# pscoro/JPEG-XL-Lossy-Image-Compression-Thesis

Hardware: AMD Instinct MI355X
Metric: MPix/s VarDCT encode @ d1.0, 8K RGB (higher is better)
Workload: dtype f32; 1 GPU; 8k 7680x4320 RGB8 (synth_rgb8), VarDCT d1 e7, cjxl defaults (JXG_FLAGS_CJXL_DEFAULTS: Gaborish + EPF + masking AQ), proposals=0, ans-coded, 1 frame(s) per step, 2 distinct frames cycled, streaming entry points (jxg_submit_rgb8_device / jxg_receive, one host thread); global_batch=1, parallelism=frame-dp1

## Files before the change

jpeg-xl-lossy-image-compression-thesis_amd/csrc/jxg_ac.hip:

```cpp
#include "jxg_device.h"
#include "jxg_kernels.h"

namespace jxg {

constexpr int kAcCtxPad = (kAcCtx + 15) & ~15;
__constant__ __attribute__((aligned(16))) uint8_t c_cluster[kAcCtxPad];

constexpr int kAcThreads = 1024;

struct GroupGeom {
  int bx0, by0, gw, gh;
};
__device__ __forceinline__ uint32_t slot_group(const uint32_t* glist, uint32_t g0, uint32_t i) {
  return glist ? glist[i] : g0 + i;
}
__device__ __forceinline__ GroupGeom group_geom(const AcArgs& a, int g) {
  GroupGeom r;
  const int gx = g % (int)a.gxs, gy = g / (int)a.gxs;
  r.bx0 = gx * 32;
  r.by0 = gy * 32;
  r.gw = min(32, (int)a.bxs - r.bx0);
  r.gh = min(32, (int)a.bys - r.by0);
  return r;
}

__device__ __forceinline__ void load_coefs(const int16_t* q, uint32_t* w) {
  const uint4* p = reinterpret_cast<const uint4*>(q);
#pragma unroll
  for (int i = 0; i < 8; i++) {
    const uint4 t = p[i];
    w[4 * i + 0] = t.x;
    w[4 * i + 1] = t.y;
    w[4 * i + 2] = t.z;
    w[4 * i + 3] = t.w;
  }
}
__device__ __forceinline__ int32_t coef(const uint32_t* w, int k) {
  return (int32_t)(int16_t)(w[k >> 1] >> ((k & 1) * 16));
}

__device__ __forceinline__ int freq_ctx(int k) {
  return k < 16 ? max(k - 1, 0) : (k < 32 ? 15 + ((k - 16) >> 1) : 23 + ((k - 32) >> 2));
}
__device__ __forceinline__ int nnz_ctx(int n) {
  return n < 2 ? 0 : n < 3 ? 31 : n < 5 ? 62 : n < 9 ? 93 : n < 13 ? 123 : n < 21 ? 152
       : n < 33 ? 180 : 206;
}

__device__ __forceinline__ int block_ctx_of(int c, int acs) {
  return kDefaultCtxMap[(c < 2 ? c ^ 1 : 2) * 13 + kStrategyOrder[acs]];
}

constexpr int kAcTok = 64;
constexpr int kEmitLdsWords = 24576;

__device__ __forceinline__ int channel_of(int ci) { return ci == 0 ? 1 : (ci == 1 ? 0 : 2); }

__device__ __forceinline__ void varblock_dims(int type, int& lcb, int& cx, int& cy) {
  switch (type) {
    case 6: lcb = 1, cx = 1, cy = 2; break;
    case 7: lcb = 1, cx = 2, cy = 1; break;
    case 4: lcb = 2, cx = 2, cy = 2; break;
    case 10: lcb = 3, cx = 2, cy = 4; break;
    case 11: lcb = 3, cx = 4, cy = 2; break;
    case 5: lcb = 4, cx = 4, cy = 4; break;
    case 19: lcb = 5, cx = 4, cy = 8; break;
    case 20: lcb = 5, cx = 8, cy = 4; break;
    case 18: lcb = 6, cx = 8, cy = 8; break;
    case 22: lcb = 7, cx = 8, cy = 16; break;
    case 23: lcb = 7, cx = 16, cy = 8; break;
    case 21: lcb = 8, cx = 16, cy = 16; break;
    case 25: lcb = 9, cx = 16, cy = 32; break;
    case 26: lcb = 9, cx = 32, cy = 16; break;
    case 24: lcb = 10, cx = 32, cy = 32; break;
    default: lcb = 0, cx = 1, cy = 1; break;
  }
}

constexpr int kBands = 4;
static_assert(kBands * kBandTokStride == kGroupTokStride, "band record spaces tile the group's");

__device__ __forceinline__ uint32_t rec_index(const uint32_t* bt, uint32_t k) {
  uint32_t j = 0, lo = 0, cum = 0;
#pragma unroll
  for (int i = 0; i < kBands - 1; i++) {
    cum += bt[i];
    const bool past = k >= cum;
    lo = past ? cum : lo;
    j += past ? 1u : 0u;
  }
  return j * (uint32_t)kBandTokStride + (k - lo);
}

struct SliceTask {
  bool valid;
  int bx, by, obx, oby, sl, lcb, cx, type;
  size_t gb, ogb;
};
__device__ __forceinline__ SliceTask slice_task(const AcArgs& a, const GroupGeom& G, int y0) {
  SliceTask t;
  const int b = threadIdx.x;
  t.bx = b & 31;
  t.by = y0 + (b >> 5);
  t.valid = t.bx < G.gw && t.by < G.gh;
  if (!t.valid) t.bx = t.by = 0;
  t.gb = (size_t)(G.by0 + t.by) * a.bxs + G.bx0 + t.bx;
  t.type = t.valid ? (a.acs[t.gb] & 0x7F) : 0;
  int cy;
  varblock_dims(t.type, t.lcb, t.cx, cy);
  t.obx = t.bx & ~(t.cx - 1);
  t.oby = t.by & ~(cy - 1);
  t.sl = (t.by - t.oby) * t.cx + (t.bx - t.obx);
  t.ogb = (size_t)(G.by0 + t.oby) * a.bxs + G.bx0 + t.obx;
  return t;
}
__device__ __forceinline__ int block_of_slice(const SliceTask& t, int j, int y0) {
  return (t.oby - y0 + j / t.cx) * 32 + t.obx + j % t.cx;
}

template <int BR>
struct AcLds {
  uint8_t nz[3][(BR + 1) * 32];
  uint8_t snz[3][BR * 32];
  uint8_t last[3][BR * 32];
  int8_t lastk[3][BR * 32];
};
__device__ __forceinline__ int predict_nz(const uint8_t* nzc, int bx, int by, int y0) {
  const int r = by - y0 + 1;
  if (bx == 0) return by == 0 ? 32 : nzc[(r - 1) * 32 + bx];
  if (by == 0) return nzc[r * 32 + bx - 1];
  return (nzc[(r - 1) * 32 + bx] + nzc[r * 32 + bx - 1] + 1) / 2;
}

template <int BR>
__device__ __forceinline__ uint32_t task_token_count(const AcArgs& a, const SliceTask& t,
                                                     const AcLds<BR>& L, int c, int y0) {
  if (t.lcb == 0) {
    uint32_t w[32];
    load_coefs(a.ac + (t.gb * 3 + c) * 64, w);
    int last = 0;
#pragma unroll
    for (int kk = 1; kk < 64; kk++) last = coef(w, kk) != 0 ? kk : last;
    return 1u + (uint32_t)last;
  }
  const int cb = 1 << t.lcb;
  int K = -1;
  for (int j = 0; j < cb; j++) {
    const int lk = L.lastk[c][block_of_slice(t, j, y0)];
    K = lk >= 0 ? j * 64 + lk : K;
  }
  const int lo = max(t.sl * 64, cb), hi = min(t.sl * 64 + 63, K);
  return (t.sl == 0 ? 1u : 0u) + (hi >= lo ? (uint32_t)(hi - lo + 1) : 0u);
}

template <int BR>
__device__ __forceinline__ void fill_slices(const AcArgs& a, const GroupGeom& G,
                                            const SliceTask& t, AcLds<BR>& L, int y0) {
  const size_t nb = (size_t)a.bxs * a.bys;
  constexpr int kPos = (BR + 1) * 32, kNT = BR * 32, kIt = (kPos + kNT - 1) / kNT;
  uint32_t acsv[kIt], nzv[kIt][3];
  bool in[kIt];
#pragma unroll
  for (int it = 0; it < kIt; it++) {
    const int i = threadIdx.x + it * kNT, r = i >> 5, bx = i & 31, by = y0 - 1 + r;
    in[it] = i < kPos && bx < G.gw && by >= 0 && by < G.gh;
    const size_t gb = in[it] ? (size_t)(G.by0 + by) * a.bxs + G.bx0 + bx : 0;
    acsv[it] = in[it] ? a.acs[gb] : 0u;
#pragma unroll
    for (int c = 0; c < 3; c++) nzv[it][c] = in[it] ? a.nz[c * nb + gb] : 0u;
  }
#pragma unroll
  for (int it = 0; it < kIt; it++) {
    if (!in[it]) continue;
    const int i = threadIdx.x + it * kNT;
    int l, cx, cy;
    varblock_dims((int)acsv[it], l, cx, cy);
#pragma unroll
    for (int c = 0; c < 3; c++) L.nz[c][i] = (uint8_t)((nzv[it][c] + (1u << l) - 1) >> l);
  }
  if (t.valid && t.lcb > 0) {
    const int cb = 1 << t.lcb, me = threadIdx.x;
#pragma unroll 1
    for (int c = 0; c < 3; c++) {
      uint32_t w[32];
      load_coefs(a.ac + (t.gb * 3 + c) * 64, w);
      int n = 0, lk = -1;
#pragma unroll
      for (int kk = 0; kk < 64; kk++) {
        const bool on = (t.sl * 64 + kk >= cb) && coef(w, kk) != 0;
        n += on;
        lk = on ? kk : lk;
      }
      L.snz[c][me] = (uint8_t)n;
      L.last[c][me] = coef(w, 63) != 0;
      L.lastk[c][me] = (int8_t)lk;
    }
  }
}

template <int BR>
__device__ __forceinline__ void slice_state(const SliceTask& t, const AcLds<BR>& L, int c, int y0,
                                            int nz, int& left, int& prev) {
  const int cb = 1 << t.lcb;
  left = nz;
  prev = nz > cb * 4 ? 0 : 1;
  if (t.sl > 0) {
    for (int j = 0; j < t.sl; j++) left -= L.snz[c][block_of_slice(t, j, y0)];
    if (t.sl * 64 - 1 >= cb) prev = L.last[c][block_of_slice(t, t.sl - 1, y0)];
  }
}

template <int NT>
__device__ __forceinline__ uint32_t block_excl_scan(uint32_t v, uint32_t* sWave,
                                                    uint32_t* total) {
  const int lane = threadIdx.x & 63, wv = threadIdx.x >> 6;
  uint32_t incl = v;
#pragma unroll
  for (int d = 1; d < 64; d <<= 1) {
    const uint32_t t = __shfl_up(incl, d);
    if (lane >= d) incl += t;
  }
  if (lane == 63) sWave[wv] = incl;
  __syncthreads();
  uint32_t before = 0, all = 0;
#pragma unroll
  for (int i = 0; i < NT / 64; i++) {
    const uint32_t x = sWave[i];
    before += i < wv ? x : 0u;
    all += x;
  }
  *total = all;
  return before + incl - v;
}

#ifdef JXG_FRONT_PROFILE
__device__ unsigned long long g_hprof[8];
#define HPROF(k)                                                     \
  do {                                                               \
    if (threadIdx.x == 0) {                                          \
      const unsigned long long now_ = __builtin_readcyclecounter();  \
      if ((k) > 0) atomicAdd(&g_hprof[(k)], now_ - hprof_t0);       \
      else atomicAdd(&g_hprof[0], 1ull);                             \
      hprof_t0 = now_;                                               \
    }                                                                \
  } while (0)
void dump_hist_profile() {
  unsigned long long h[8];
  if (hipMemcpyFromSymbol(h, HIP_SYMBOL(g_hprof), sizeof(h)) != hipSuccess) return;
  static const char* kNames[6] = {"workgroups", "fill slices", "token counts", "scan", "walk", "flush"};
  std::fprintf(stderr, "ac_hist thread-0 shader cycles (Mcycles summed over workgroups):\n");
  for (int k = 0; k < 6; k++) std::fprintf(stderr, "  %-16s %12.3f\n", kNames[k], k ? h[k] / 1e6 : (double)h[0]);
}
#else
#define HPROF(k) \
  do {           \
  } while (0)
void dump_hist_profile() {}
#endif
template <int BR>
__global__ __launch_bounds__(BR * 32) void ac_hist_kernel(Batch<AcArgs> bt_) {
  constexpr int kBandBlocks = BR * 32, kHistThreads = kBandBlocks, kWgBands = 32 / BR;
  const AcArgs& a = bt_.a[blockIdx.z];
  constexpr bool kWide = BR == 32;
  constexpr int kHistWords = kWide ? kMaxClusters * kAcTok : kMaxClusters * kAcTok / 2;
  __shared__ uint32_t sHist[kHistWords];
  __shared__ AcLds<BR> L;
  __shared__ __attribute__((aligned(16))) uint8_t sClu[kAcCtxPad];
  __shared__ uint32_t sTask[3][kBandBlocks];
  __shared__ uint32_t sBase[kBandBlocks];
  __shared__ uint32_t sWave[kHistThreads / 64];
  __shared__ uint32_t sBound, sNtok[3];
  __shared__ uint16_t sNnzCtx[64];
  __shared__ uint8_t sFreqCtx[64];
  const uint32_t slot = blockIdx.x / kWgBands, band = blockIdx.x % kWgBands;
  const int g = (int)slot_group(a.glist, a.g0, slot);
  const GroupGeom G = group_geom(a, g);
  const int y0 = (int)band * BR;
  if (BR == 32 && threadIdx.x > 0 && threadIdx.x < kBands)
    a.bandtok[g * kBands + threadIdx.x] = 0;
  if (y0 >= G.gh) {
    if (threadIdx.x == 0) a.bandtok[g * kBands + band] = 0;
    return;
  }
#ifdef JXG_FRONT_PROFILE
  unsigned long long hprof_t0 = 0;
#endif
  HPROF(0);
  for (int i = threadIdx.x; i < kHistWords; i += blockDim.x) sHist[i] = 0;
  if (threadIdx.x < 64) {
    sNnzCtx[threadIdx.x] = (uint16_t)nnz_ctx(threadIdx.x);
    sFreqCtx[threadIdx.x] = (uint8_t)freq_ctx(threadIdx.x);
  }
  {
    constexpr int kQ = kAcCtxPad / 16, kQIt = (kQ + kHistThreads - 1) / kHistThreads;
    uint4 q[kQIt];
#pragma unroll
    for (int it = 0; it < kQIt; it++) {
      const int i = threadIdx.x + it * kHistThreads;
      q[it] = i < kQ ? reinterpret_cast<const uint4*>(c_cluster)[i] : make_uint4(0, 0, 0, 0);
    }
#pragma unroll
    for (int it = 0; it < kQIt; it++) {
      const int i = threadIdx.x + it * kHistThreads;
      if (i < kQ) reinterpret_cast<uint4*>(sClu)[i] = q[it];
    }
  }
  if (threadIdx.x < 3) sNtok[threadIdx.x] = 0;
  if (threadIdx.x == 0) sBound = 0;
  const SliceTask t = slice_task(a, G, y0);
  uint32_t nzo[3];
#pragma unroll
  for (int c = 0; c < 3; c++) nzo[c] = t.valid ? a.nz[c * (size_t)a.bxs * a.bys + t.ogb] : 0u;
  fill_slices(a, G, t, L, y0);
  __syncthreads();
  HPROF(1);
  const int me = threadIdx.x;
  if (t.valid) {
#pragma unroll 1
    for (int ci = 0; ci < 3; ci++) sTask[ci][me] = task_token_count(a, t, L, channel_of(ci), y0);
  }
  __syncthreads();
  HPROF(2);
  uint32_t vtot = 0;
  const int cb = 1 << t.lcb;
  if (t.valid && t.sl == 0) {
    for (int ci = 0; ci < 3; ci++)
      for (int j = 0; j < cb; j++) vtot += sTask[ci][block_of_slice(t, j, y0)];
  }
  uint32_t total;
  const uint32_t off = block_excl_scan<kHistThreads>(vtot, sWave, &total);
  if (t.valid && t.sl == 0) sBase[me] = off;
  __syncthreads();
  HPROF(3);
  uint32_t bound = 0, nt[3] = {0, 0, 0};
  uint32_t* rec = a.tokens + (uint64_t)slot * kGroupTokStride + (uint64_t)band * kBandTokStride;
  uint32_t pos = t.valid ? sBase[(t.oby - y0) * 32 + t.obx] : 0u;
  const int lane = threadIdx.x & 63;
  const uint64_t below = lane ? (~0ull >> (64 - lane)) : 0ull;
  auto hist_add = [&](uint32_t clu, uint32_t tok) {
    const uint32_t bin = clu * kAcTok + tok;
    if (kWide)
      atomicAdd(&sHist[bin], 1u);
    else
      atomicAdd(&sHist[bin >> 1], 1u << ((bin & 1u) * 16u));
  };
#pragma unroll 1
  for (int ci = 0; ci < 3; ci++) {
    const int c = channel_of(ci);
    uint32_t idx = 0, cnt = 0, info = 0, info2 = 0, tok0 = 0;
    if (t.valid) {
      uint32_t before = 0, chan_total = 0;
      for (int j = 0; j < cb; j++) {
        const uint32_t b = sTask[ci][block_of_slice(t, j, y0)];
        before += j < t.sl ? b : 0u;
        chan_total += b;
      }
      idx = pos + before;
      cnt = sTask[ci][me];
      pos += chan_total;
      const int nz = (int)nzo[c];
      int left, prev;
      slice_state(t, L, c, y0, nz, left, prev);
      const int bctx = block_ctx_of(c, t.type);
      info = (uint32_t)left | ((uint32_t)prev << 16) | ((uint32_t)t.lcb << 17) |
             ((uint32_t)bctx << 21);
      info2 = (uint32_t)t.sl;
      if (t.sl == 0) {
        const int pred = predict_nz(L.nz[c], t.bx, t.by, y0);
        uint32_t tok, nb, bits;
        hybrid420((uint32_t)nz, tok, nb, bits);
        const uint32_t clu = sClu[nz_bucket(pred) * kBlockCtx + bctx];
        hist_add(clu, tok);
        bound += 15u + nb;
        tok0 = clu | (tok << 8) | (nb << 14) | (bits << 18);
        rec[idx] = tok0;
      }
      nt[0] += c == 0 ? cnt : 0u;
      nt[1] += c == 1 ? cnt : 0u;
      nt[2] += c == 2 ? cnt : 0u;
    }
    const bool need = t.valid && cnt > (t.sl == 0 ? 1u : 0u);
    const uint32_t qoff = (uint32_t)((t.gb * 3 + c) * 64);
    uint64_t M = __ballot(need);
#ifndef JXG_AC_BATCH
#define JXG_AC_BATCH 8
#endif
    constexpr int kBatch = JXG_AC_BATCH;
    while (M) {
      int js[kBatch];
#pragma unroll
      for (int u = 0; u < kBatch; u++) {
        js[u] = M ? (int)__builtin_ctzll(M) : -1;
        M = M ? M & (M - 1) : 0ull;
      }
      int32_t v8[kBatch];
#pragma unroll
      for (int u = 0; u < kBatch; u++)
        v8[u] = js[u] >= 0 ? a.ac[(uint32_t)__builtin_amdgcn_readlane((int)qoff, js[u]) + lane] : 0;
#pragma unroll
      for (int u = 0; u < kBatch; u++) {
        if (js[u] < 0) break;
        const int j = js[u];
        const uint32_t ij = (uint32_t)__builtin_amdgcn_readlane((int)info, j);
        const uint32_t idxj = (uint32_t)__builtin_amdgcn_readlane((int)idx, j);
        const int slj = __builtin_amdgcn_readlane((int)info2, j), lcbj = (ij >> 17) & 15;
        const int leftj = ij & 0xFFFF, prevj = (ij >> 16) & 1, bctxj = ij >> 21;
        const int cbj = 1 << lcbj;
        const int k = slj * 64 + lane;
        const int lo = max(slj * 64, cbj);
        const int32_t v = v8[u];
        const bool on = k >= cbj;
        const uint64_t m = __ballot(on && v != 0);
        const int left_k = leftj - __popcll(m & below);
        if (on && left_k > 0) {
          const int prev_k = k == lo ? prevj : (int)((m >> (lane - 1)) & 1);
          const int ctx = kBlockCtx * kNzBuckets + kZdCtx * bctxj +
                          (sNnzCtx[(left_k + cbj - 1) >> lcbj] + sFreqCtx[k >> lcbj]) * 2 + prev_k;
          uint32_t tok, nb, bits;
          hybrid420(pack_signed(v), tok, nb, bits);
          const uint32_t clu = sClu[ctx];
          hist_add(clu, tok);
          bound += 15u + nb;
          rec[idxj + (slj == 0 ? 1u : 0u) + (uint32_t)(k - lo)] =
              clu | (tok << 8) | (nb << 14) | (bits << 18);
        }
      }
    }
  }
  atomicAdd(&sBound, bound);
  atomicAdd(&sNtok[0], nt[0]);
  atomicAdd(&sNtok[1], nt[1]);
  atomicAdd(&sNtok[2], nt[2]);
  __syncthreads();
  HPROF(4);
  for (int i = threadIdx.x; i < kHistWords; i += blockDim.x) {
    const uint32_t w = sHist[i];
    if (!w) continue;
    if (kWide) {
      atomicAdd(&a.hist[(i / kAcTok) * kAlpha + (i % kAcTok)], w);
      continue;
    }
    const int bin = 2 * i;
    if (w & 0xFFFFu) atomicAdd(&a.hist[(bin / kAcTok) * kAlpha + (bin % kAcTok)], w & 0xFFFFu);
    if (w >> 16) atomicAdd(&a.hist[((bin + 1) / kAcTok) * kAlpha + ((bin + 1) % kAcTok)], w >> 16);
  }
  if (threadIdx.x == 0) {
    atomicAdd(&a.bound[g], sBound);
    atomicAdd(&a.ntok[g * 3 + 0], sNtok[0]);
    atomicAdd(&a.ntok[g * 3 + 1], sNtok[1]);
    atomicAdd(&a.ntok[g * 3 + 2], sNtok[2]);
    a.bandtok[g * kBands + band] = total;
  }
  HPROF(5);
}

__device__ __forceinline__ uint32_t wave_incl_scan(uint32_t v) {
  const int lane = threadIdx.x & 63;
#pragma unroll
  for (int d = 1; d < 64; d <<= 1) {
    const uint32_t t = __shfl_up(v, d);
    if (lane >= d) v += t;
  }
  return v;
}
__global__ __launch_bounds__(kAcThreads) void ac_emit_kernel(AcArgs a) {
  __shared__ uint32_t sCode[kMaxClusters * kAcTok];
  __shared__ __attribute__((aligned(16))) uint32_t sBits[kEmitLdsWords];
  __shared__ uint32_t sWave[kAcThreads / 64];
  const int g = (int)slot_group(a.glist, a.g0, blockIdx.x);
  for (int i = threadIdx.x; i < kMaxClusters * kAcTok; i += blockDim.x)
    sCode[i] = a.codes[(i / kAcTok) * kAlpha + (i % kAcTok)];
  for (int i = threadIdx.x; i < kEmitLdsWords / 4; i += blockDim.x)
    reinterpret_cast<uint4*>(sBits)[i] = make_uint4(0, 0, 0, 0);
  const uint32_t n = a.ntok[g * 3] + a.ntok[g * 3 + 1] + a.ntok[g * 3 + 2];
  const uint32_t* rec = a.tokens + (uint64_t)blockIdx.x * kGroupTokStride;
  uint32_t bt[kBands];
#pragma unroll
  for (int i = 0; i < kBands; i++) bt[i] = a.bandtok[g * kBands + i];
  constexpr int kWaves = kAcThreads / 64;
  const int lane = threadIdx.x & 63, wv = threadIdx.x >> 6;
  const uint32_t chunk = ((n + kWaves * 64 - 1) / (kWaves * 64)) * 64;
  const uint32_t lo = min(n, wv * chunk), hi = min(n, lo + chunk);
  __syncthreads();
  auto code_of = [&](uint32_t r) { return sCode[(r & 0xFF) * kAcTok + ((r >> 8) & 63)]; };
  uint32_t tot = 0;
  for (uint32_t k = lo + lane; k < hi; k += 64) {
    const uint32_t r = rec[rec_index(bt, k)];
    tot += (code_of(r) >> 16) + ((r >> 14) & 15);
  }
#pragma unroll
  for (int d = 32; d > 0; d >>= 1) tot += __shfl_xor(tot, d, 64);
  if (lane == 0) sWave[wv] = tot;
  __syncthreads();
  uint32_t run = 0, total = 0;
#pragma unroll
  for (int i = 0; i < kWaves; i++) {
    const uint32_t x = sWave[i];
    run += i < wv ? x : 0u;
    total += x;
  }
  const uint64_t base = a.base[g];
  const bool lds = total <= (uint32_t)kEmitLdsWords * 32u;
  if (!lds) {
    for (uint32_t i = threadIdx.x; i < (total + 31) / 32; i += blockDim.x) a.scratch[(base >> 5) + i] = 0;
    __threadfence();
    __syncthreads();
  }
  uint32_t* buf = lds ? sBits : a.scratch;
  const uint64_t bias = lds ? 0 : base;
  for (uint32_t k0 = lo; k0 < hi; k0 += 64) {
    const uint32_t k = k0 + lane;
    uint32_t len = 0, val = 0;
    if (k < hi) {
      const uint32_t r = rec[rec_index(bt, k)], cl = code_of(r);
      len = (cl >> 16) + ((r >> 14) & 15);
      val = (cl & 0xFFFFu) | ((r >> 18) << (cl >> 16));
    }
    const uint32_t incl = wave_incl_scan(len);
    if (len) {
      const uint64_t pos = bias + run + incl - len;
      const uint64_t w = pos >> 5;
      const uint32_t sh = (uint32_t)(pos & 31);
      atomicOr(&buf[w], val << sh);
      if (sh + len > 32) atomicOr(&buf[w + 1], val >> (32 - sh));
    }
    run += __shfl(incl, 63, 64);
  }
  if (lds) {
    __syncthreads();
    const uint32_t nw = (total + 31) / 32;
    uint32_t* dst = a.scratch + (base >> 5);
    for (uint32_t i = threadIdx.x; i < nw; i += blockDim.x) dst[i] = sBits[i];
  }
  if (threadIdx.x == 0) a.bits[g] = total;
}

constexpr int kAnsWgWaves = 8;
constexpr int kAnsHelpers = 6;
constexpr int kAnsPieces = (64 + kAnsHelpers - 1) / kAnsHelpers;
constexpr int kAnsBlk = 64;
constexpr int kAnsRow = 65;
constexpr uint32_t kAnsIdle = kAnsHists * 64;
struct AnsConst {
  double rcp;
  uint32_t nf2;
  uint32_t base2;
};
struct AnsChainP {
  int n;
  uint32_t slot;
  uint32_t c1, c2, c3;
  uint32_t g;
  uint32_t pad[2];
};
struct AnsLds {
  AnsConst c[kAnsIdle + 1];
  uint16_t ent[256];
  uint32_t inv[kAnsHists * 4096 / 2];
  uint32_t ea[2][kAnsBlk * kAnsRow];
  uint32_t x[2][kAnsBlk * kAnsRow];
  AnsChainP ch[64];
  int T;
};
__device__ __forceinline__ void ans_chain(const AnsArgs& a, uint32_t blk) {
  __shared__ __attribute__((aligned(16))) AnsLds L;
  const uint32_t c0 = blk * 64;
  if (c0 >= a.n) return;
  const uint32_t* src = reinterpret_cast<const uint32_t*>(a.tab);
  for (uint32_t i = threadIdx.x; i < a.nhist * 512; i += blockDim.x)
    reinterpret_cast<uint4*>(L.inv)[i] = reinterpret_cast<const uint4*>(src + kAnsInvOff / 4)[i];
  for (uint32_t i = threadIdx.x; i <= kAnsIdle; i += blockDim.x) {
    uint32_t f = 4096, row = 0;
    if (i < a.nhist * 64) {
      const uint32_t e = src[(i >> 6) * 128 + (i & 63)];
      f = (e & 0xFFF) + 1;
      row = (i >> 6) * 4096 + (e >> 12);
    }
    L.c[i].rcp = 1.0 / (double)f;
    L.c[i].nf2 = (uint32_t)(-(int)(2 * f));
    L.c[i].base2 = 2 * row;
  }
  for (uint32_t i = threadIdx.x; i < 256; i += blockDim.x)
    L.ent[i] = (uint16_t)(i < 136 ? min((uint32_t)a.tab[kAnsMapOff + i], kAnsHists - 1) * 64 * 16
                                  : kAnsIdle * 16);
  const uint32_t lane = threadIdx.x & 63, wave = threadIdx.x >> 6;
  if (wave == 0) {
    AnsChainP P = {0, 0, 0, 0, 0, ~0u, {0, 0}};
    if (c0 + lane < a.n) {
      P.slot = a.order[c0 + lane];
      P.g = slot_group(a.glist, a.g0, P.slot);
      P.n = (int)(a.ntok[P.g * 3] + a.ntok[P.g * 3 + 1] + a.ntok[P.g * 3 + 2]);
      P.c1 = a.bandtok[P.g * kBands];
      P.c2 = P.c1 + a.bandtok[P.g * kBands + 1];
      P.c3 = P.c2 + a.bandtok[P.g * kBands + 2];
    }
    L.ch[lane] = P;
    int m = P.n;
#pragma unroll
    for (int d = 32; d > 0; d >>= 1) m = max(m, __shfl_xor(m, d, 64));
    if (lane == 0) L.T = m + 1;
  }
  __syncthreads();
  const int NB = (L.T + kAnsBlk - 1) / kAnsBlk;
  const uint8_t* inv = reinterpret_cast<const uint8_t*>(L.inv);
  const uint8_t* cst = reinterpret_cast<const uint8_t*>(L.c);
  const int h = (wave & 3) ? (int)(wave >> 2) * 3 + (int)(wave & 3) - 1 : -1;
  const uint32_t hs = lane;
  auto word_of = [&](uint32_t rec) {
    return ((uint32_t)L.ent[rec & 0xFF] + ((rec >> 4) & 0x3F0)) | ((rec >> 14) & 15) | (rec >> 18) << 14;
  };
  auto record = [&](const AnsChainP& P, int i) {
    const uint32_t u = (uint32_t)i;
    const uint32_t j = (u >= P.c1 ? 1u : 0u) + (u >= P.c2 ? 1u : 0u) + (u >= P.c3 ? 1u : 0u);
    const uint32_t lo = u >= P.c3 ? P.c3 : u >= P.c2 ? P.c2 : u >= P.c1 ? P.c1 : 0u;
    return a.tokens[(uint64_t)P.slot * kGroupTokStride + j * (uint32_t)kBandTokStride + (u - lo)];
  };
  constexpr uint32_t kIdleRec = 0xFFu;
  auto fetch = [&](int b, uint32_t* R) {
#pragma unroll
    for (int j = 0; j < kAnsPieces; j++) {
      const int q = h + kAnsHelpers * j;
      R[j] = kIdleRec;
      if (q < 64) {
        const AnsChainP P = L.ch[q];
        const int i = P.n - 1 - (b * kAnsBlk + (int)hs);
        if (i >= 0) R[j] = record(P, i);
      }
    }
  };
  auto fill = [&](int b, const uint32_t* R) {
#pragma unroll
    for (int j = 0; j < kAnsPieces; j++) {
      const int q = h + kAnsHelpers * j;
      if (q < 64) L.ea[b & 1][hs * kAnsRow + q] = word_of(R[j]);
    }
  };
  auto unstage = [&](int b, uint32_t* X, uint32_t* RC) {
#pragma unroll
    for (int j = 0; j < kAnsPieces; j++) {
      const int q = h + kAnsHelpers * j;
      X[j] = RC[j] = 0;
      if (q < 64) {
        X[j] = L.x[b & 1][hs * kAnsRow + q];
        RC[j] = L.ea[b & 1][hs * kAnsRow + q];
      }
    }
  };
  auto flush = [&](int b, const uint32_t* X, const uint32_t* RC) {
#pragma unroll
    for (int j = 0; j < kAnsPieces; j++) {
      const int q = h + kAnsHelpers * j;
      if (q < 64) {
        const AnsChainP P = L.ch[q];
        const int i = P.n - 1 - (b * kAnsBlk + (int)hs);
        const uint32_t x = X[j], w = RC[j];
        if (i >= 0) {
          const uint32_t nf2 = reinterpret_cast<const AnsConst*>(cst + (w & 0x3FF0))->nf2;
          const bool em = (x >> 12) >= (uint32_t)__mul24((int)nf2, -128);
          const uint32_t raw = w >> 14, nb = w & 15;
          const uint64_t o = (uint64_t)P.slot * kGroupTokStride + (uint32_t)i;
          a.val[o] = em ? (x & 0xFFFFu) | raw << 16 : raw;
          a.len[o] = (uint8_t)(em ? nb + 16 : nb);
        } else if (i == -1 && P.g != ~0u) {
          a.state[P.g] = x;
        }
      }
    }
  };
  uint32_t k = 0x130u, v = 0;
  auto chain_block = [&](int b) {
    const uint32_t* eas = L.ea[b & 1] + lane;
    uint32_t* xo = L.x[b & 1] + lane;
    AnsConst Cn = *reinterpret_cast<const AnsConst*>(cst + (eas[0] & 0x3FF0));
#pragma unroll
    for (int s = 0; s < kAnsBlk; s++) {
      const AnsConst C = Cn;
      if (s + 1 < kAnsBlk) Cn = *reinterpret_cast<const AnsConst*>(cst + (eas[(s + 1) * kAnsRow] & 0x3FF0));
      const double hr = 0.5 * C.rcp;
      const uint32_t Fq = (uint32_t)__mul24((int)C.nf2, -128);
      const uint32_t sh = k >= Fq ? 16u : 0u;
      const uint32_t x = (k << 12) + v;
      const uint32_t xs = x >> sh;
      const uint32_t kk = (uint32_t)__builtin_fma((double)xs, C.rcp, hr);
      const uint32_t x2 = (xs << 1) + C.base2;
      uint32_t addr;
      asm("v_mad_i32_i24 %0, %1, %2, %3" : "=v"(addr) : "v"(kk), "v"(C.nf2), "v"(x2));
      v = *reinterpret_cast<const uint16_t*>(inv + addr);
      k = kk;
      xo[s * kAnsRow] = x;
    }
  };
  if (wave == 0) __builtin_amdgcn_s_setprio(3);
  uint32_t R[kAnsPieces], X[kAnsPieces], RC[kAnsPieces];
  if (h >= 0) {
    fetch(0, R);
    fill(0, R);
    fetch(1, R);
  }
  __syncthreads();
  for (int b = 0; b < NB; b++) {
    if (wave == 0) {
      chain_block(b);
    } else if (h >= 0) {
      if (b > 0) unstage(b - 1, X, RC);
      fill(b + 1, R);
      fetch(b + 2, R);
      if (b > 0) flush(b - 1, X, RC);
    }
    __syncthreads();
  }
  if (h >= 0) {
    unstage(NB - 1, X, RC);
    flush(NB - 1, X, RC);
  }
}
__global__ __launch_bounds__(kAnsWgWaves * 64) void ans_encode_kernel(Batch<AnsArgs> bt_) {
  ans_chain(bt_.a[blockIdx.z], blockIdx.x);
}
constexpr int kAnsDiagWaves = 8;
__device__ __forceinline__ uint32_t wave_ror1(uint32_t x) {
  return (uint32_t)__builtin_amdgcn_mov_dpp((int)x, 0x13C, 0xF, 0xF, false);
}
__device__ __forceinline__ void ans_chain_diag(const AnsArgs& a, uint32_t blk) {
  __shared__ uint32_t sSym[kAnsHists * 128];
  __shared__ uint32_t sInv[kAnsHists * 4096 / 2];
  __shared__ uint8_t sMap[136];
  const uint32_t* src = reinterpret_cast<const uint32_t*>(a.tab);
  for (uint32_t i = threadIdx.x; i < a.nhist * 128; i += blockDim.x) sSym[i] = src[i];
  for (uint32_t i = threadIdx.x; i < a.nhist * 2048; i += blockDim.x)
    sInv[i] = src[kAnsInvOff / 4 + i];
  for (uint32_t i = threadIdx.x; i < 136; i += blockDim.x) sMap[i] = a.tab[kAnsMapOff + i];
  __syncthreads();
  const uint8_t* inv = reinterpret_cast<const uint8_t*>(sInv);
  const uint32_t lane = threadIdx.x & 63;
  const uint32_t gi = __builtin_amdgcn_readfirstlane(blk * kAnsDiagWaves + (threadIdx.x >> 6));
  if (gi >= a.n) return;
  const uint32_t slot = __builtin_amdgcn_readfirstlane(a.order[gi]);
  const uint32_t g = __builtin_amdgcn_readfirstlane(slot_group(a.glist, a.g0, slot));
  __builtin_amdgcn_s_setprio(3);
  const int n = (int)(a.ntok[g * 3] + a.ntok[g * 3 + 1] + a.ntok[g * 3 + 2]);
  const uint64_t b = (uint64_t)slot * kGroupTokStride;
  uint32_t bt[kBands];
#pragma unroll
  for (int i = 0; i < kBands; i++) bt[i] = a.bandtok[g * kBands + i];
  uint32_t k = 0x130u, v = 0;
  uint32_t rec = (int)lane < min(64, n) ? a.tokens[b + rec_index(bt, n - 1 - lane)] : 0u;
  for (int hi = n; hi > 0; hi -= 64) {
    const int cnt = min(64, hi);
    uint32_t f = 4096, base2 = 0;
    if ((int)lane < cnt) {
      const uint32_t h = sMap[rec & 0xFF], e = sSym[h * 128 + ((rec >> 8) & 63)];
      f = (e & 0xFFF) + 1;
      base2 = 2 * (h * 4096 + (e >> 12));
    }
    const uint32_t Fq = f << 8;
    const uint32_t nf2 = (uint32_t)(-(int)(2 * f));
    const double rcp = 1.0 / (double)f, hr = 0.5 * rcp;
    const int hn = hi - 64;
    const uint32_t nrec = (int)lane < min(64, hn) ? a.tokens[b + rec_index(bt, hn - 1 - lane)] : 0u;
    uint32_t X = 0;
    uint32_t xin = 0;
    auto step = [&](int s) {
      const uint32_t kin = wave_ror1(k);
      const uint32_t sh = kin >= Fq ? 16u : 0u;
      if (s > 0)
        asm("v_cndmask_b32_e64 %0, %1, %2, %3" : "=v"(X) : "v"(X), "v"(xin), "s"(1ull << (s - 1)));
      __builtin_amdgcn_sched_barrier(0);
      const uint32_t vin = wave_ror1(v);
      const uint32_t x = (kin << 12) + vin;
      const uint32_t xs = x >> sh;
      const uint32_t kk = (uint32_t)__builtin_fma((double)xs, rcp, hr);
      const uint32_t x2 = (xs << 1) + base2;
      uint32_t addr;
      asm("v_mad_i32_i24 %0, %1, %2, %3" : "=v"(addr) : "v"(kk), "v"(nf2), "v"(x2));
      v = *reinterpret_cast<const uint16_t*>(inv + addr);
      k = kk;
      xin = x;
      __builtin_amdgcn_sched_barrier(0);
    };
    if (cnt == 64) {
#pragma unroll
      for (int s = 0; s < 64; s++) step(s);
      asm("v_cndmask_b32_e64 %0, %1, %2, %3" : "=v"(X) : "v"(X), "v"(xin), "s"(1ull << 63));
    } else {
      for (int s = 0; s < cnt; s++) {
        const uint32_t kin = wave_ror1(k);
        const bool emit = kin >= Fq;
        const uint32_t t = (kin << 12) >> (emit ? 16 : 0);
        const double P = __builtin_fma((double)t, rcp, hr);
        const uint32_t C = 2 * t + base2;
        const uint32_t vin = wave_ror1(v);
        X = (int)lane == s ? (kin << 12) + vin : X;
        const uint32_t vv = emit ? 0u : vin;
        const uint32_t kk = (uint32_t)__builtin_fma((double)vv, rcp, P);
        const uint32_t addr = (uint32_t)((int)(2 * vv + C) - (int)(2 * f) * (int)kk);
        v = *reinterpret_cast<const uint16_t*>(inv + addr);
        k = kk;
      }
    }
    if ((int)lane < cnt) {
      const bool em = (X >> 20) >= f;
      const uint32_t raw = rec >> 18, nb = (rec >> 14) & 15;
      a.val[b + hi - 1 - lane] = em ? (X & 0xFFFFu) | raw << 16 : raw;
      a.len[b + hi - 1 - lane] = (uint8_t)(em ? nb + 16 : nb);
    }
    rec = nrec;
    if (hi <= 64) {
      const uint32_t kf = __builtin_amdgcn_readlane(k, cnt - 1);
      const uint32_t vf = __builtin_amdgcn_readlane(v, cnt - 1);
      if (lane == 0) a.state[g] = (kf << 12) + vf;
    }
  }
  if (n == 0 && lane == 0) a.state[g] = 0x130000u;
}
__global__ __launch_bounds__(kAnsDiagWaves * 64) void ans_encode_diag_kernel(Batch<AnsArgs> bt_) {
  ans_chain_diag(bt_.a[blockIdx.z], blockIdx.x);
}
constexpr int kSumThreads = 1024;
__global__ __launch_bounds__(kSumThreads) void ans_sums_kernel(Batch<AnsArgs> bt_) {
  __shared__ uint32_t sC[kAnsMaxChunks];
  __shared__ uint32_t sTot[kSumThreads / 64];
  const AnsArgs& a = bt_.a[blockIdx.z];
  const uint32_t slot = blockIdx.x;
  if (slot >= a.n) return;
  const uint32_t g = slot_group(a.glist, a.g0, slot);
  const uint32_t n = a.ntok[g * 3] + a.ntok[g * 3 + 1] + a.ntok[g * 3 + 2];
  const uint32_t K = (n + 63) / 64;
  const uint64_t b = (uint64_t)slot * kGroupTokStride;
  const int lane = threadIdx.x & 63, wv = threadIdx.x >> 6;
  for (uint32_t q = threadIdx.x; q < K; q += kSumThreads) sC[q] = 0;
  __syncthreads();
  const uint32_t off = (64u - (n & 63u)) & 63u, r = n & 15u;
  const uint4* L = reinterpret_cast<const uint4*>(a.len + b);
  for (uint32_t w = threadIdx.x; w < (n + 15) / 16; w += kSumThreads) {
    const uint4 v = L[w];
    const uint32_t d[4] = {v.x, v.y, v.z, v.w};
    const uint32_t valid = min(16u, n - 16u * w);
    uint32_t lo = 0, hi = 0;
#pragma unroll
    for (uint32_t j = 0; j < 16; j++) {
      const uint32_t x = j < valid ? (d[j >> 2] >> (8 * (j & 3))) & 0xFFu : 0u;
      if (j < r) lo += x;
      else hi += x;
    }
    if (lo) atomicAdd(&sC[(16u * w + off) >> 6], lo);
    if (hi) atomicAdd(&sC[(16u * w + r + off) >> 6], hi);
  }
  __syncthreads();
  uint32_t* csum = a.csum + (uint64_t)slot * kAnsMaxChunks;
  uint32_t tot = 0;
  for (uint32_t q = threadIdx.x; q < K; q += kSumThreads) {
    const uint32_t c = sC[q];
    csum[q] = c;
    tot += c;
  }
#pragma unroll
  for (int m = 32; m > 0; m >>= 1) tot += __shfl_xor(tot, m, 64);
  if (lane == 0) sTot[wv] = tot;
  __syncthreads();
  uint32_t total = 32;
#pragma unroll
  for (int i = 0; i < kSumThreads / 64; i++) total += sTot[i];
  if (threadIdx.x == 0) a.bits[g] = total;
  uint32_t* dst = a.scratch + (a.base[g] >> 5);
  for (uint32_t i = threadIdx.x; i < (total + 31) / 32; i += kSumThreads) dst[i] = 0;
}
constexpr int kSegChunks = 64, kEmitThreads = 256;
constexpr int kSegWords = (kSegChunks * 64 * 29 + 31) / 32 + 2;
__global__ __launch_bounds__(kEmitThreads) void ans_emit_kernel(Batch<AnsArgs> bt_) {
  __shared__ __attribute__((aligned(16))) uint32_t sBits[kSegWords];
  __shared__ uint32_t sCs[kSegChunks + 1];
  __shared__ uint32_t sPre[kEmitThreads / 64];
  const AnsArgs& a = bt_.a[blockIdx.z];
  const uint32_t slot = blockIdx.x, seg = blockIdx.y;
  if (slot >= a.n) return;
  const uint32_t g = slot_group(a.glist, a.g0, slot);
  const uint32_t n = a.ntok[g * 3] + a.ntok[g * 3 + 1] + a.ntok[g * 3 + 2];
  const uint32_t K = (n + 63) / 64, q0 = seg * kSegChunks;
  const uint64_t base = a.base[g];
  if (seg == 0 && threadIdx.x == 0) a.scratch[base >> 5] = a.state[g];
  if (q0 >= K) return;
  const uint32_t q1 = min(K, q0 + kSegChunks);
  const uint32_t* csum = a.csum + (uint64_t)slot * kAnsMaxChunks;
  const int lane = threadIdx.x & 63, wv = threadIdx.x >> 6;
  uint32_t pre = 0;
  for (uint32_t q = threadIdx.x; q < q0; q += kEmitThreads) pre += csum[q];
#pragma unroll
  for (int d = 32; d > 0; d >>= 1) pre += __shfl_xor(pre, d, 64);
  if (lane == 0) sPre[wv] = pre;
  if (threadIdx.x <= kSegChunks) sCs[threadIdx.x] = q0 + threadIdx.x < q1 ? csum[q0 + threadIdx.x] : 0u;
  for (int i = threadIdx.x; i < kSegWords; i += kEmitThreads) sBits[i] = 0;
  __syncthreads();
  const uint64_t start = base + 32 + sPre[0] + sPre[1] + sPre[2] + sPre[3];
  const uint32_t sh0 = (uint32_t)(start & 31);
  uint32_t segbits = 0;
  for (uint32_t q = 0; q < q1 - q0; q++) segbits += sCs[q];
  auto chunk_lo = [&](uint32_t q) { return q == 0 ? 0u : n - 64u * (K - q); };
  const uint64_t b = (uint64_t)slot * kGroupTokStride;
  constexpr int kPerWave = kSegChunks / (kEmitThreads / 64);
  uint32_t run = sh0;
  for (int i = 0; i < wv * kPerWave; i++) run += sCs[i];
  for (int i = 0; i < kPerWave; i++) {
    const uint32_t q = q0 + (uint32_t)(wv * kPerWave + i);
    if (q >= q1) break;
    const uint32_t lo = chunk_lo(q), hi = chunk_lo(q + 1);
    const uint32_t k = lo + (uint32_t)lane;
    const uint32_t len = k < hi ? a.len[b + k] : 0u;
    const uint32_t val = k < hi ? a.val[b + k] : 0u;
    const uint32_t incl = wave_incl_scan(len);
    if (len) {
      const uint32_t pos = run + incl - len;
      const uint32_t w = pos >> 5, sh = pos & 31;
      atomicOr(&sBits[w], val << sh);
      if (sh + len > 32) atomicOr(&sBits[w + 1], val >> (32 - sh));
    }
    run += sCs[wv * kPerWave + i];
  }
  __syncthreads();
  const uint32_t nw = (sh0 + segbits + 31) / 32;
  uint32_t* dst = a.scratch + (start >> 5);
  for (uint32_t i = threadIdx.x; i < nw; i += kEmitThreads) {
    const uint32_t v = sBits[i];
    if (i == 0 || i == nw - 1) {
      if (v) atomicOr(&dst[i], v);
    } else {
      dst[i] = v;
    }
  }
}

void launch_ans(const AnsArgs* a, uint32_t k, hipStream_t s, bool streamed) {
  if (!k || !a[0].n) return;
  const Batch<AnsArgs> b = make_batch(a, k);
  uint32_t n = 0, maxtok = 0;
  for (uint32_t i = 0; i < k; i++) {
    n = max(n, a[i].n);
    maxtok = max(maxtok, a[i].max_tokens);
  }
  if (streamed)
    hipLaunchKernelGGL(ans_encode_kernel, dim3((n + 63) / 64, 1, k), dim3(kAnsWgWaves * 64), 0, s, b);
  else
    hipLaunchKernelGGL(ans_encode_diag_kernel, dim3((n + kAnsDiagWaves - 1) / kAnsDiagWaves, 1, k),
                       dim3(kAnsDiagWaves * 64), 0, s, b);
  hipLaunchKernelGGL(ans_sums_kernel, dim3(n, 1, k), dim3(kSumThreads), 0, s, b);
  const uint32_t nseg = (maxtok + kSegChunks * 64 - 1) / (kSegChunks * 64);
  if (nseg) hipLaunchKernelGGL(ans_emit_kernel, dim3(n, nseg, k), dim3(kEmitThreads), 0, s, b);
}

void launch_ac_hist(const AcArgs* a, uint32_t k, uint32_t ngroups, hipStream_t s, bool whole_group) {
  if (!ngroups || !k) return;
  if (whole_group)
    hipLaunchKernelGGL(ac_hist_kernel<32>, dim3(ngroups, 1, k), dim3(1024), 0, s, make_batch(a, k));
  else
    hipLaunchKernelGGL(ac_hist_kernel<8>, dim3(ngroups * kBands, 1, k), dim3(256), 0, s, make_batch(a, k));
}
void launch_ac_emit(const AcArgs& a, uint32_t ngroups, hipStream_t s) {
  if (ngroups) hipLaunchKernelGGL(ac_emit_kernel, dim3(ngroups), dim3(kAcThreads), 0, s, a);
}
hipError_t set_cluster_table(const uint8_t* tab, hipStream_t s) {
  return hipMemcpyToSymbolAsync(HIP_SYMBOL(c_cluster), tab, kAcCtx, 0, hipMemcpyHostToDevice, s);
}

}
```

Measured before the change: 10750 MPix/s.

## Use per-slice nonzero bitmasks and compacted token-level work distribution in AC histogram

Replaces the per-slice count, last and lastk LDS arrays with one 64-bit nonzero mask per slice, so token counts and context state come from clz and popcount. This drops the separate token-count pass and one barrier. The walk now compacts the active slices in each wave, prefix-sums their token counts, and hands one token to each lane through ds_permute/bpermute with LDS head bitmaps, so lanes stay busy instead of idling on sparse slices. It also reuses LDS through a union, narrows the scan base to 16 bits for narrow bands, sets occupancy hints in launch_bounds and lowers the batch size. In exchange the inner loop adds cross-lane shuffles and wave-level LDS syncs, which adds complexity and risk.

```diff
diff --git a/jpeg-xl-lossy-image-compression-thesis_amd/csrc/jxg_ac.hip b/jpeg-xl-lossy-image-compression-thesis_amd/csrc/jxg_ac.hip
--- a/jpeg-xl-lossy-image-compression-thesis_amd/csrc/jxg_ac.hip
+++ b/jpeg-xl-lossy-image-compression-thesis_amd/csrc/jxg_ac.hip
@@ -121,9 +121,7 @@
 template <int BR>
 struct AcLds {
   uint8_t nz[3][(BR + 1) * 32];
-  uint8_t snz[3][BR * 32];
-  uint8_t last[3][BR * 32];
-  int8_t lastk[3][BR * 32];
+  uint64_t mask[3][BR * 32];
 };
 __device__ __forceinline__ int predict_nz(const uint8_t* nzc, int bx, int by, int y0) {
   const int r = by - y0 + 1;
@@ -132,25 +130,35 @@
   return (nzc[(r - 1) * 32 + bx] + nzc[r * 32 + bx - 1] + 1) / 2;
 }
 
+__device__ __forceinline__ uint64_t slice_mask(const int16_t* q, int first) {
+  uint32_t w[32];
+  load_coefs(q, w);
+  uint32_t m0 = 0, m1 = 0;
+#pragma unroll
+  for (int kk = 0; kk < 32; kk++) {
+    m0 |= coef(w, kk) != 0 ? 1u << kk : 0u;
+    m1 |= coef(w, kk + 32) != 0 ? 1u << kk : 0u;
+  }
+  const uint64_t m = (uint64_t)m0 | ((uint64_t)m1 << 32);
+  return first >= 64 ? 0ull : m & (~0ull << first);
+}
+
 template <int BR>
-__device__ __forceinline__ uint32_t task_token_count(const AcArgs& a, const SliceTask& t,
-                                                     const AcLds<BR>& L, int c, int y0) {
-  if (t.lcb == 0) {
-    uint32_t w[32];
-    load_coefs(a.ac + (t.gb * 3 + c) * 64, w);
-    int last = 0;
-#pragma unroll
-    for (int kk = 1; kk < 64; kk++) last = coef(w, kk) != 0 ? kk : last;
-    return 1u + (uint32_t)last;
-  }
+__device__ __forceinline__ int varblock_last(const SliceTask& t, const AcLds<BR>& L, int c, int y0) {
   const int cb = 1 << t.lcb;
   int K = -1;
   for (int j = 0; j < cb; j++) {
-    const int lk = L.lastk[c][block_of_slice(t, j, y0)];
-    K = lk >= 0 ? j * 64 + lk : K;
-  }
-  const int lo = max(t.sl * 64, cb), hi = min(t.sl * 64 + 63, K);
-  return (t.sl == 0 ? 1u : 0u) + (hi >= lo ? (uint32_t)(hi - lo + 1) : 0u);
+    const uint64_t m = L.mask[c][block_of_slice(t, j, y0)];
+    K = m ? j * 64 + 63 - (int)__builtin_clzll(m) : K;
+  }
+  return K;
+}
+__device__ __forceinline__ uint32_t slice_coef_tokens(int K, int cb, int sl) {
+  const int lo = max(sl * 64, cb), hi = min(sl * 64 + 63, K);
+  return hi >= lo ? (uint32_t)(hi - lo + 1) : 0u;
+}
+__device__ __forceinline__ uint32_t tokens_before_slice(int K, int cb, int sl) {
+  return sl == 0 ? 0u : 1u + (uint32_t)max(0, min(sl * 64 - 1, K) - cb + 1);
 }
 
 template <int BR>
@@ -178,23 +186,11 @@
 #pragma unroll
     for (int c = 0; c < 3; c++) L.nz[c][i] = (uint8_t)((nzv[it][c] + (1u << l) - 1) >> l);
   }
-  if (t.valid && t.lcb > 0) {
-    const int cb = 1 << t.lcb, me = threadIdx.x;
+  if (t.valid) {
+    const int first = max((1 << t.lcb) - t.sl * 64, 0);
 #pragma unroll 1
-    for (int c = 0; c < 3; c++) {
-      uint32_t w[32];
-      load_coefs(a.ac + (t.gb * 3 + c) * 64, w);
-      int n = 0, lk = -1;
-#pragma unroll
-      for (int kk = 0; kk < 64; kk++) {
-        const bool on = (t.sl * 64 + kk >= cb) && coef(w, kk) != 0;
-        n += on;
-        lk = on ? kk : lk;
-      }
-      L.snz[c][me] = (uint8_t)n;
-      L.last[c][me] = coef(w, 63) != 0;
-      L.lastk[c][me] = (int8_t)lk;
-    }
+    for (int c = 0; c < 3; c++)
+      L.mask[c][threadIdx.x] = slice_mask(a.ac + (t.gb * 3 + c) * 64, first);
   }
 }
 
@@ -205,8 +201,8 @@
   left = nz;
   prev = nz > cb * 4 ? 0 : 1;
   if (t.sl > 0) {
-    for (int j = 0; j < t.sl; j++) left -= L.snz[c][block_of_slice(t, j, y0)];
-    if (t.sl * 64 - 1 >= cb) prev = L.last[c][block_of_slice(t, t.sl - 1, y0)];
+    for (int j = 0; j < t.sl; j++) left -= __popcll(L.mask[c][block_of_slice(t, j, y0)]);
+    if (t.sl * 64 - 1 >= cb) prev = (int)(L.mask[c][block_of_slice(t, t.sl - 1, y0)] >> 63);
   }
 }
 
@@ -257,8 +253,19 @@
   } while (0)
 void dump_hist_profile() {}
 #endif
+
+#ifndef JXG_AC_BATCH
+#define JXG_AC_BATCH 6
+#endif
+constexpr int kAcBatch = JXG_AC_BATCH;
+
+__device__ __forceinline__ void wave_lds_sync() {
+  __builtin_amdgcn_fence(__ATOMIC_SEQ_CST, "wavefront");
+  __builtin_amdgcn_wave_barrier();
+}
+
 template <int BR>
-__global__ __launch_bounds__(BR * 32) void ac_hist_kernel(Batch<AcArgs> bt_) {
+__global__ __launch_bounds__(BR * 32, BR == 8 ? 5 : 4) void ac_hist_kernel(Batch<AcArgs> bt_) {
   constexpr int kBandBlocks = BR * 32, kHistThreads = kBandBlocks, kWgBands = 32 / BR;
   const AcArgs& a = bt_.a[blockIdx.z];
   constexpr bool kWide = BR == 32;
@@ -266,12 +273,18 @@
   __shared__ uint32_t sHist[kHistWords];
   __shared__ AcLds<BR> L;
   __shared__ __attribute__((aligned(16))) uint8_t sClu[kAcCtxPad];
-  __shared__ uint32_t sTask[3][kBandBlocks];
-  __shared__ uint32_t sBase[kBandBlocks];
-  __shared__ uint32_t sWave[kHistThreads / 64];
-  __shared__ uint32_t sBound, sNtok[3];
-  __shared__ uint16_t sNnzCtx[64];
-  __shared__ uint8_t sFreqCtx[64];
+  using BaseT = typename std::conditional<kWide, uint32_t, uint16_t>::type;
+  union ScanOrHeads {
+    BaseT base[kBandBlocks];
+    unsigned long long head[kHistThreads / 64][kAcBatch];
+  };
+  __shared__ ScanOrHeads sU;
+  BaseT* const sBase = sU.base;
+  unsigned long long(*const sHead)[kAcBatch] = sU.head;
+  static_assert(sizeof(sU.head) <= sizeof(sU.base), "heads fit into the base array");
+  __shared__ uint32_t sWave[kHistThreads / 64 < 4 ? 4 : kHistThreads / 64];
+  uint32_t* const sAcc = sWave;
+  __shared__ uint8_t sNnzCtx[64], sFreqCtx[64];
   const uint32_t slot = blockIdx.x / kWgBands, band = blockIdx.x % kWgBands;
   const int g = (int)slot_group(a.glist, a.g0, slot);
   const GroupGeom G = group_geom(a, g);
@@ -288,7 +301,7 @@
   HPROF(0);
   for (int i = threadIdx.x; i < kHistWords; i += blockDim.x) sHist[i] = 0;
   if (threadIdx.x < 64) {
-    sNnzCtx[threadIdx.x] = (uint16_t)nnz_ctx(threadIdx.x);
+    sNnzCtx[threadIdx.x] = (uint8_t)nnz_ctx(threadIdx.x);
     sFreqCtx[threadIdx.x] = (uint8_t)freq_ctx(threadIdx.x);
   }
   {
@@ -305,8 +318,6 @@
       if (i < kQ) reinterpret_cast<uint4*>(sClu)[i] = q[it];
     }
   }
-  if (threadIdx.x < 3) sNtok[threadIdx.x] = 0;
-  if (threadIdx.x == 0) sBound = 0;
   const SliceTask t = slice_task(a, G, y0);
   uint32_t nzo[3];
 #pragma unroll
@@ -315,28 +326,30 @@
   __syncthreads();
   HPROF(1);
   const int me = threadIdx.x;
+  const int cb = 1 << t.lcb;
+  int K0 = -1, K1 = -1, K2 = -1;
+  uint32_t vtot = 0;
   if (t.valid) {
-#pragma unroll 1
-    for (int ci = 0; ci < 3; ci++) sTask[ci][me] = task_token_count(a, t, L, channel_of(ci), y0);
-  }
-  __syncthreads();
+    K0 = varblock_last(t, L, channel_of(0), y0);
+    K1 = varblock_last(t, L, channel_of(1), y0);
+    K2 = varblock_last(t, L, channel_of(2), y0);
+    if (t.sl == 0)
+      vtot = 3u + (uint32_t)(max(0, K0 - cb + 1) + max(0, K1 - cb + 1) + max(0, K2 - cb + 1));
+  }
   HPROF(2);
-  uint32_t vtot = 0;
-  const int cb = 1 << t.lcb;
-  if (t.valid && t.sl == 0) {
-    for (int ci = 0; ci < 3; ci++)
-      for (int j = 0; j < cb; j++) vtot += sTask[ci][block_of_slice(t, j, y0)];
-  }
   uint32_t total;
   const uint32_t off = block_excl_scan<kHistThreads>(vtot, sWave, &total);
-  if (t.valid && t.sl == 0) sBase[me] = off;
+  if (t.valid && t.sl == 0) sBase[me] = (BaseT)off;
   __syncthreads();
   HPROF(3);
-  uint32_t bound = 0, nt[3] = {0, 0, 0};
+  uint32_t bound = 0;
   uint32_t* rec = a.tokens + (uint64_t)slot * kGroupTokStride + (uint64_t)band * kBandTokStride;
   uint32_t pos = t.valid ? sBase[(t.oby - y0) * 32 + t.obx] : 0u;
-  const int lane = threadIdx.x & 63;
+  if (threadIdx.x < 4) sAcc[threadIdx.x] = 0;
+  __syncthreads();
+  const int lane = threadIdx.x & 63, wv = threadIdx.x >> 6;
   const uint64_t below = lane ? (~0ull >> (64 - lane)) : 0ull;
+  const uint32_t gbw = (uint32_t)((G.by0 + y0 + 2 * wv) * (int)a.bxs + G.bx0);
   auto hist_add = [&](uint32_t clu, uint32_t tok) {
     const uint32_t bin = clu * kAcTok + tok;
     if (kWide)
@@ -347,24 +360,19 @@
 #pragma unroll 1
   for (int ci = 0; ci < 3; ci++) {
     const int c = channel_of(ci);
-    uint32_t idx = 0, cnt = 0, info = 0, info2 = 0, tok0 = 0;
+    uint32_t ncoef = 0, info = 0, xrec = 0;
     if (t.valid) {
-      uint32_t before = 0, chan_total = 0;
-      for (int j = 0; j < cb; j++) {
-        const uint32_t b = sTask[ci][block_of_slice(t, j, y0)];
-        before += j < t.sl ? b : 0u;
-        chan_total += b;
-      }
-      idx = pos + before;
-      cnt = sTask[ci][me];
-      pos += chan_total;
+      const int K = ci == 0 ? K0 : (ci == 1 ? K1 : K2);
+      ncoef = slice_coef_tokens(K, cb, t.sl);
+      const uint32_t idx = pos + tokens_before_slice(K, cb, t.sl);
+      pos += 1u + (uint32_t)max(0, K - cb + 1);
       const int nz = (int)nzo[c];
       int left, prev;
       slice_state(t, L, c, y0, nz, left, prev);
       const int bctx = block_ctx_of(c, t.type);
       info = (uint32_t)left | ((uint32_t)prev << 16) | ((uint32_t)t.lcb << 17) |
              ((uint32_t)bctx << 21);
-      info2 = (uint32_t)t.sl;
+      xrec = (idx + (t.sl == 0 ? 1u : 0u)) | ((uint32_t)t.sl << 18);
       if (t.sl == 0) {
         const int pred = predict_nz(L.nz[c], t.bx, t.by, y0);
         uint32_t tok, nb, bits;
@@ -372,65 +380,81 @@
         const uint32_t clu = sClu[nz_bucket(pred) * kBlockCtx + bctx];
         hist_add(clu, tok);
         bound += 15u + nb;
-        tok0 = clu | (tok << 8) | (nb << 14) | (bits << 18);
-        rec[idx] = tok0;
+        rec[idx] = clu | (tok << 8) | (nb << 14) | (bits << 18);
       }
-      nt[0] += c == 0 ? cnt : 0u;
-      nt[1] += c == 1 ? cnt : 0u;
-      nt[2] += c == 2 ? cnt : 0u;
-    }
-    const bool need = t.valid && cnt > (t.sl == 0 ? 1u : 0u);
-    const uint32_t qoff = (uint32_t)((t.gb * 3 + c) * 64);
-    uint64_t M = __ballot(need);
-#ifndef JXG_AC_BATCH
-#define JXG_AC_BATCH 8
-#endif
-    constexpr int kBatch = JXG_AC_BATCH;
-    while (M) {
-      int js[kBatch];
-#pragma unroll
-      for (int u = 0; u < kBatch; u++) {
-        js[u] = M ? (int)__builtin_ctzll(M) : -1;
-        M = M ? M & (M - 1) : 0ull;
+      atomicAdd(&sAcc[1 + c], ncoef + (t.sl == 0 ? 1u : 0u));
+    }
+    const uint64_t NM = __ballot(ncoef != 0);
+    if (NM == 0) continue;
+    const int nne = __popcll(NM);
+    uint32_t incl = ncoef;
+#pragma unroll
+    for (int d = 1; d < 64; d <<= 1) {
+      const uint32_t x = __shfl_up(incl, d);
+      if (lane >= d) incl += x;
+    }
+    const uint32_t T = (uint32_t)__builtin_amdgcn_readlane((int)incl, 63);
+    const int dest = (ncoef ? __popcll(NM & below) : nne + __popcll(~NM & below)) << 2;
+    const uint32_t cS = (uint32_t)__builtin_amdgcn_ds_permute(
+        dest, (int)((incl - ncoef) | ((uint32_t)lane << 12) | ((t.sl == 0 ? (uint32_t)cb : 0u) << 18)));
+    const uint32_t cI = (uint32_t)__builtin_amdgcn_ds_permute(dest, (int)info);
+    const uint32_t cX = (uint32_t)__builtin_amdgcn_ds_permute(dest, (int)xrec);
+    const uint32_t cE = (uint32_t)__builtin_amdgcn_ds_permute(dest, (int)(incl - 1u));
+    uint32_t tb = 0;
+#pragma unroll 1
+    for (uint32_t p0 = 0; p0 * 64 < T; p0 += kAcBatch) {
+      if (lane < kAcBatch) sHead[wv][lane] = 0ull;
+      wave_lds_sync();
+      {
+        const uint32_t w = (cE >> 6) - p0;
+        if (lane < nne && w < (uint32_t)kAcBatch) atomicOr(&sHead[wv][w], 1ull << (cE & 63u));
       }
-      int32_t v8[kBatch];
-#pragma unroll
-      for (int u = 0; u < kBatch; u++)
-        v8[u] = js[u] >= 0 ? a.ac[(uint32_t)__builtin_amdgcn_readlane((int)qoff, js[u]) + lane] : 0;
-#pragma unroll
-      for (int u = 0; u < kBatch; u++) {
-        if (js[u] < 0) break;
-        const int j = js[u];
-        const uint32_t ij = (uint32_t)__builtin_amdgcn_readlane((int)info, j);
-        const uint32_t idxj = (uint32_t)__builtin_amdgcn_readlane((int)idx, j);
-        const int slj = __builtin_amdgcn_readlane((int)info2, j), lcbj = (ij >> 17) & 15;
+      wave_lds_sync();
+      uint32_t sv[kAcBatch];
+      int32_t v8[kAcBatch];
+#pragma unroll
+      for (int u = 0; u < kAcBatch; u++) {
+        const unsigned long long hv = sHead[wv][u];
+        const uint32_t e0 = (uint32_t)__builtin_amdgcn_readfirstlane((int)(uint32_t)hv);
+        const uint32_t e1 = (uint32_t)__builtin_amdgcn_readfirstlane((int)(uint32_t)(hv >> 32));
+        const uint32_t r = (tb + __builtin_amdgcn_mbcnt_hi(e1, __builtin_amdgcn_mbcnt_lo(e0, 0u))) & 63u;
+        tb += (uint32_t)(__popc(e0) + __popc(e1));
+        sv[u] = (uint32_t)__builtin_amdgcn_ds_bpermute((int)(r << 2), (int)cS) | (r << 24);
+        const uint32_t flat = (p0 + u) * 64 + lane, j = (sv[u] >> 12) & 63u;
+        const uint32_t kloc = ((sv[u] >> 18) & 63u) + flat - (sv[u] & 4095u);
+        const uint32_t gb = gbw + (j >> 5) * a.bxs + (j & 31u);
+        v8[u] = flat < T ? a.ac[(gb * 3 + c) * 64 + kloc] : 0;
+      }
+#pragma unroll
+      for (int u = 0; u < kAcBatch; u++) {
+        if ((p0 + u) * 64 >= T) break;
+        const int ra = (int)((sv[u] >> 22) & 0xFCu);
+        const uint32_t ij = (uint32_t)__builtin_amdgcn_ds_bpermute(ra, (int)cI);
+        const uint32_t xj = (uint32_t)__builtin_amdgcn_ds_bpermute(ra, (int)cX);
+        const uint32_t flat = (p0 + u) * 64 + lane, j = (sv[u] >> 12) & 63u;
+        const uint32_t offk = flat - (sv[u] & 4095u);
+        const int kloc = (int)(((sv[u] >> 18) + offk) & 63u);
+        const uint64_t m = L.mask[c][wv * 64 + j];
+        const int slj = xj >> 18, lcbj = (ij >> 17) & 15;
         const int leftj = ij & 0xFFFF, prevj = (ij >> 16) & 1, bctxj = ij >> 21;
-        const int cbj = 1 << lcbj;
-        const int k = slj * 64 + lane;
-        const int lo = max(slj * 64, cbj);
-        const int32_t v = v8[u];
-        const bool on = k >= cbj;
-        const uint64_t m = __ballot(on && v != 0);
-        const int left_k = leftj - __popcll(m & below);
-        if (on && left_k > 0) {
-          const int prev_k = k == lo ? prevj : (int)((m >> (lane - 1)) & 1);
+        const int k = slj * 64 + kloc;
+        const int left_k = leftj - __popcll(m & ((1ull << kloc) - 1ull));
+        if (flat < T && left_k > 0) {
+          const int32_t v = v8[u];
+          const int prev_k = offk == 0 ? prevj : (int)((m >> ((kloc - 1) & 63)) & 1);
           const int ctx = kBlockCtx * kNzBuckets + kZdCtx * bctxj +
-                          (sNnzCtx[(left_k + cbj - 1) >> lcbj] + sFreqCtx[k >> lcbj]) * 2 + prev_k;
+                          (sNnzCtx[(left_k + (1 << lcbj) - 1) >> lcbj] + sFreqCtx[k >> lcbj]) * 2 + prev_k;
           uint32_t tok, nb, bits;
           hybrid420(pack_signed(v), tok, nb, bits);
           const uint32_t clu = sClu[ctx];
           hist_add(clu, tok);
           bound += 15u + nb;
-          rec[idxj + (slj == 0 ? 1u : 0u) + (uint32_t)(k - lo)] =
-              clu | (tok << 8) | (nb << 14) | (bits << 18);
+          rec[(xj & 0x3FFFFu) + offk] = clu | (tok << 8) | (nb << 14) | (bits << 18);
         }
       }
     }
   }
-  atomicAdd(&sBound, bound);
-  atomicAdd(&sNtok[0], nt[0]);
-  atomicAdd(&sNtok[1], nt[1]);
-  atomicAdd(&sNtok[2], nt[2]);
+  atomicAdd(&sAcc[0], bound);
   __syncthreads();
   HPROF(4);
   for (int i = threadIdx.x; i < kHistWords; i += blockDim.x) {
@@ -445,10 +469,10 @@
     if (w >> 16) atomicAdd(&a.hist[((bin + 1) / kAcTok) * kAlpha + ((bin + 1) % kAcTok)], w >> 16);
   }
   if (threadIdx.x == 0) {
-    atomicAdd(&a.bound[g], sBound);
-    atomicAdd(&a.ntok[g * 3 + 0], sNtok[0]);
-    atomicAdd(&a.ntok[g * 3 + 1], sNtok[1]);
-    atomicAdd(&a.ntok[g * 3 + 2], sNtok[2]);
+    atomicAdd(&a.bound[g], sAcc[0]);
+    atomicAdd(&a.ntok[g * 3 + 0], sAcc[1]);
+    atomicAdd(&a.ntok[g * 3 + 1], sAcc[2]);
+    atomicAdd(&a.ntok[g * 3 + 2], sAcc[3]);
     a.bandtok[g * kBands + band] = total;
   }
   HPROF(5);
```

Measured after the change: 10830 MPix/s (median of 6 runs). Within noise of the previous version (+0.8%).
